# RazonIn4K/image-restoration-platform

Hardware: AMD Instinct MI355X
Metric: restored images/sec @1024x1024 bs=8 (higher is better)
Workload: dtype bf16; 1 GPU; 1024x1024 RGB u8, batch 8 per GPU: fused classifier scan + RestoreNet-v0 (43 convs, 779.9 GFLOP/image), seeded random-init weights; global_batch=8, parallelism=per-image data parallel x1, no collective, streams=1

## Files before the change

### image_restoration_platform_amd/build.py

```python
import concurrent.futures
import os
import subprocess
import sys

HERE = os.path.dirname(os.path.abspath(__file__))
CSRC = os.path.join(HERE, "csrc")
OBJ = os.path.join(HERE, "build")
LIB = os.path.join(HERE, "lib", "libire.so")

SOURCES = [
    ("classifier.hip", ["-ffp-contract=off"] + (["-DCLS_ABL=" + os.environ["CLS_ABL"]] if os.environ.get("CLS_ABL") else [])),
    ("conv_mfma.hip", []),
    ("conv_rb.hip", (["-DIRE_RB_ABLATE"] if os.environ.get("IRE_RB_ABLATE") else []) +
     (["-DIRE_RB_NGP64=" + os.environ["IRE_RB_NGP64"]] if os.environ.get("IRE_RB_NGP64") else [])),
    ("conv_w4.hip", (["-DIRE_W4_STAMPS"] if os.environ.get("IRE_RB_ABLATE") else []) +
     (["-DIRE_W4_TICKS"] if os.environ.get("IRE_RB_ABLATE") == "2" else []) +
     (["-DW4_TEPI=" + os.environ["IRE_W4_TEPI"]] if os.environ.get("IRE_W4_TEPI") else []) +
     (["-DIRE_W4_TL"] if os.environ.get("IRE_W4_TL") else [])),
    ("conv_up.hip", (["-DIRE_UP_ABL=" + os.environ["IRE_UP_ABL"]] if os.environ.get("IRE_UP_ABL") else []) +
     (["-DIRE_UP_D=" + os.environ["IRE_UP_D"]] if os.environ.get("IRE_UP_D") else []) +
     (["-DIRE_UP_TEPI=" + os.environ["IRE_UP_TEPI"]] if os.environ.get("IRE_UP_TEPI") else [])),
    ("conv_upq.hip", os.environ.get("UQ_DEFS", "").split()),
    ("conv_dnq.hip", os.environ.get("DQ_DEFS", "").split()),
    ("conv_down.hip", (["-DDN_LD_NT=" + os.environ["DN_LD_NT"]] if os.environ.get("DN_LD_NT") else [])),
    ("conv_stem.hip", []),
    ("conv_f8.hip", []),
    ("conv_pc.hip", (["-DC3_ABL=" + os.environ["C3_ABL"]] if os.environ.get("C3_ABL") else []) +
     (["-DC3_PRIO=" + os.environ["C3_PRIO"]] if os.environ.get("C3_PRIO") else []) +
     (["-DC3_RES_PRE=" + os.environ["C3_RES_PRE"]] if os.environ.get("C3_RES_PRE") else []) +
     (["-DC3_TEPI=" + os.environ["C3_TEPI"]] if os.environ.get("C3_TEPI") else []) +
     (["-DC3_TEPI64=" + os.environ["C3_TEPI64"]] if os.environ.get("C3_TEPI64") else []) +
     (["-DIRE_LD_ONCE32=" + os.environ["IRE_LD_ONCE32"]] if os.environ.get("IRE_LD_ONCE32") else []) +
     (["-DC3_PROD8=" + os.environ["C3_PROD8"]] if os.environ.get("C3_PROD8") else []) +
     (["-DIRE_PC_TICKS"] if os.environ.get("IRE_RB_ABLATE") == "2" else []) + (["-DIRE_W4_TL"] if os.environ.get("IRE_W4_TL") else [])),
    ("conv_pk.hip", (["-DPK_ABL=" + os.environ["PK_ABL"]] if os.environ.get("PK_ABL") else []) +
     (["-DPK_TICKS"] if os.environ.get("PK_TICKS") else []) + (["-DIRE_W4_TL"] if os.environ.get("IRE_W4_TL") else []) + os.environ.get("PK_DEFS", "").split()),
    ("gn.hip", []),
    ("fusion.hip", (["-DFUSE_FL=" + os.environ["FUSE_FL"]] if os.environ.get("FUSE_FL") else [])),
    ("preprocess.hip", []),
    ("encode.hip", []),
    ("deflate.hip", []),
    ("jpeg.hip", []),
    ("jpeg_dec.hip", []),
    ("engine.cpp", []),
    ("strips.cpp", []),
    ("api.cpp", []),
]
COMMON = ["--offload-arch=gfx950", "-O3", "-std=c++17", "-fPIC", "-Wall", "-Wno-unused-function",
          "-D__HIP_PLATFORM_AMD__"] + ([] if os.environ.get("IRE_SLP") == "1" else ["-fno-slp-vectorize"]) + \
         (["-DIRE_ST_LINE=" + os.environ["IRE_ST_LINE"]] if os.environ.get("IRE_ST_LINE") else []) + \
         (["-DIRE_ST_PART=" + os.environ["IRE_ST_PART"]] if os.environ.get("IRE_ST_PART") else []) + \
         (["-DIRE_LD_ONCE=" + os.environ["IRE_LD_ONCE"]] if os.environ.get("IRE_LD_ONCE") else []) + \
         (["-DIRE_LD_IN=" + os.environ["IRE_LD_IN"]] if os.environ.get("IRE_LD_IN") else []) + \
         os.environ.get("IRE_XFLAGS", "").split()

def _hipcc():
    for c in (os.environ.get("HIPCC"), "/opt/rocm/bin/hipcc", "hipcc"):
        if c and (os.path.isabs(c) and os.path.exists(c) or not os.path.isabs(c)):
            return c
    raise RuntimeError("hipcc not found")


def _deps_mtime():
    m = 0.0
    for root, _, files in os.walk(CSRC):
        for f in files:
# ... 94 lines not shown
```

### image_restoration_platform_amd/csrc/conv_mfma.hpp

```cpp
#pragma once
#include "common.hpp"
#include "conv_kind.hpp"

#ifndef IRE_ST_LINE
#define IRE_ST_LINE 16
#endif
#ifndef IRE_LD_ONCE
#define IRE_LD_ONCE 2
#endif
#ifndef IRE_LD_IN
#define IRE_LD_IN 0
#endif
#ifndef IRE_ST_PART
#define IRE_ST_PART 0
#endif

#include <cstdlib>

namespace ire {

inline int persistent_grid_cus() {
    static const int forced = [] { const char* v = std::getenv("IRE_GRID_CUS"); return v ? std::atoi(v) : 0; }();
    int dev = 0, cus = 256;
    (void)hipGetDevice(&dev);
// ... 8 lines not shown
    const void* in1;
    int cin0, cin1;
    int kc_split;
    int nkc;
    const unsigned short* w;
    const unsigned short* w1;
    const float* bias;
    const float2* ab;
    const float* gn_stats;
    int gn_parts, gn_hw;
    const float* gn_gamma;
    const float* gn_beta;
    const float* gn_film;
    int gn_film_stride, gn_film_off;
    float2* ab_w;
    const unsigned short* resid;
    unsigned short* out;
    const unsigned char* u8_in;
    unsigned char* u8_out;
    float* stats;
    int Hin, Win, Hout, Wout, cout;
    int tiles_x, tiles_y, nimg, nblocks;
    int group_size;
    int prio_young;
    int in_rows;
    int in_row_off;
    int iy_lo, iy_span;
    int fp8;
    const float* oscale;
    int w4_nt;
    const void* zeros;
    unsigned long long* stamps;
    int walk_rev;
};

void conv_launch(ConvKind kind, const ConvArgs& a, hipStream_t stream);

void conv_rb_launch(bool resid, bool fused_act, const ConvArgs& a, hipStream_t stream);
void conv_w4_launch(bool resid, const ConvArgs& a, hipStream_t stream);
void conv_f8_launch(bool resid, const ConvArgs& a, hipStream_t stream);
void conv_stem_launch(const ConvArgs& a, hipStream_t stream);
void conv_down_launch(const ConvArgs& a, hipStream_t stream);
void conv_head_launch(const ConvArgs& a, hipStream_t stream);
void conv_pc_launch(bool resid, bool head, const ConvArgs& a, hipStream_t stream);
void conv_pk_launch(bool resid, const ConvArgs& a, hipStream_t stream);
void conv_up_subpixel_launch(const ConvArgs& a, hipStream_t stream);
void conv_upq_launch(const ConvArgs& a, hipStream_t stream);
void conv_dnq_launch(const ConvArgs& a, hipStream_t stream);
void conv_up_launch(const ConvArgs& a, hipStream_t stream);

}
```

### image_restoration_platform_amd/csrc/conv_pc.hip

```cpp
#include "conv_mfma.hpp"
#include "conv_plan.hpp"
#include "gn_fold.hpp"
#include "persist.hpp"

#include <type_traits>

namespace ire {

namespace {

typedef __bf16 bf16x8_t __attribute__((ext_vector_type(8)));
typedef __bf16 bf16x2_t __attribute__((ext_vector_type(2)));
typedef float f32x2_t __attribute__((ext_vector_type(2)));
typedef float f32x16_t __attribute__((ext_vector_type(16)));
typedef unsigned u32x4_t __attribute__((ext_vector_type(4)));

#ifndef C3_RES_PRE
#define C3_RES_PRE -1
#endif
#ifndef C3_SCALAR
#define C3_SCALAR 1
#endif
#ifndef C3_PRIO
#define C3_PRIO 1
#endif
#ifndef C3_TEPI
#define C3_TEPI 1
#endif
#ifndef IRE_LD_ONCE32
#define IRE_LD_ONCE32 2
#endif
#ifndef C3_TEPI64
#define C3_TEPI64 1
#endif
#ifndef C3_PROD8
#define C3_PROD8 0
#endif
#ifndef C3_INTERIOR
#define C3_INTERIOR 0
#endif
#ifndef C3_ABL
#define C3_ABL 0
#endif
constexpr int C3_CONS = 512, C3_PROD = 256, C3_THREADS = C3_CONS + C3_PROD;
constexpr int pc_prod(int C, bool head) { return (C3_PROD8 && C == 32 && !head) ? 512 : 256; }
constexpr int C3_TH = 16, C3_TW = 32, C3_IH = C3_TH + 2, C3_IW = C3_TW + 2;
constexpr int C3_IN_CHUNKS = C3_IH * C3_IW * 4;
constexpr int C3_P_ITERS = (C3_IN_CHUNKS + C3_PROD - 1) / C3_PROD;
constexpr int C3_IN_BYTES = C3_P_ITERS * C3_PROD * 16;
template <int C> struct PcCfg {
    static constexpr int NT = C < 64 ? 32 : 64;
    static constexpr int NBLK = C / NT;
    static constexpr int NKC = C / 32;
    static constexpr int NTL = NT / 32;
    static constexpr int W_STAGE = 36 * NT * 16;
    static constexpr int W_STAGE_CHUNKS = 36 * NT;
    static constexpr int W_LDS = NKC * W_STAGE;
    static constexpr int W_OFF = 2 * C3_IN_BYTES;
    static constexpr int BIAS_OFF = W_OFF + W_LDS;
    static constexpr int NCC = NT / 8;
    static constexpr int RED_OFF = BIAS_OFF + C * 4;
    static constexpr int RED_HALF = 8 * NCC * 4;
    static constexpr int COEF_IMGS = pc_coef_imgs(C);
    static constexpr int COEF_OFF = RED_OFF + 2 * RED_HALF * 4;
    static constexpr int HEAD_OFF = COEF_OFF + COEF_IMGS * C * 2 * 4;
    static constexpr int PATCH_OFF = HEAD_OFF + (C == 32 ? 8 * 2 * 2 * 96 : 0);
    static constexpr int CNT_OFF = PATCH_OFF + (C == 32 ? 8 * 2048 : 0);
    static constexpr int LDS = CNT_OFF + (C == 64 ? 16 : 0);
    static_assert(LDS <= 160 * 1024, "LDS");
};

__device__ __forceinline__ unsigned c3_pack(float a, float b) {
// ... 57 lines not shown
    const int n_items = cursor.my_items;
    if (n_items == 0) return;
    const int n_stages = n_items * NKC;
    tl(0);
    {
        const unsigned char* ws = reinterpret_cast<const unsigned char*>(a.w);
        const unsigned wl = (unsigned)(size_t)(__attribute__((address_space(3))) unsigned char*)smem + K::W_OFF;
        constexpr int PIECES = NKC * K::W_STAGE_CHUNKS / 64;
        static_assert((NKC * K::W_STAGE_CHUNKS) % 64 == 0, "whole wave-instructions");
        const int wv = __builtin_amdgcn_readfirstlane(wave);
        for (int p = wv; p < PIECES; p += THREADS / 64) c3_glds16(ws + ((size_t)p * 64 + lane) * 16, wl + p * 1024);
    }
    if (a.gn_stats) gn_fold(a, smem, cursor.first_img, cursor.last_img, 512, reinterpret_cast<float2*>(smem + K::COEF_OFF));
    tl(1);

    {
        if (tid < C) reinterpret_cast<float*>(smem + K::BIAS_OFF)[tid] = a.bias[tid];
        if constexpr (C == 64) { if (tid == 0) *reinterpret_cast<unsigned*>(smem + K::CNT_OFF) = 0u; }
        const int nim = cursor.last_img - cursor.first_img + 1;
        const float2* ab = a.ab + (size_t)cursor.first_img * C;
        float2* cd = reinterpret_cast<float2*>(smem + K::COEF_OFF);
        if (!a.gn_stats) for (int i = tid; i < nim * C; i += THREADS) cd[i] = ab[i];
    }
    asm volatile("s_waitcnt vmcnt(0)" ::: "memory");
    __syncthreads();
    tl(2);

    if (__builtin_amdgcn_readfirstlane(wave) >= 8) {
#if C3_PRIO
        if (C3_PRIO != 1 || C != 32 || HEAD) asm volatile("s_setprio %0" :: "n"(C3_PRIO));
#endif
        const int tp = tid - C3_CONS;
        const int c8 = tp & 3;
        int rel[P_ITERS], lds_off[P_ITERS];
        unsigned pyx[P_ITERS];
#pragma unroll
        for (int i = 0; i < P_ITERS; ++i) {
            const int q = tp + i * PROD;
            const int p = q >> 2;
            const int py = p / C3_IW, px = p - py * C3_IW;
            pyx[i] = ((unsigned)py << 8) | (unsigned)px;
            rel[i] = (py * a.Win + px) * (2 * C) + c8 * 16;
            lds_off[i] = (p * 4 + (c8 ^ ((p >> 2) & 3))) * 16;
        }
        uint4 R[P_ITERS];
        unsigned okbits = 0;
        float cA[8], cB[8];
        PersistStage ls = cursor.cur;
        auto load_chunk = [&](int i) __attribute__((always_inline)) {
            const PersistItem& lit = ls.it;
            const int oy1 = lit.ty * C3_TH - 1, ox1 = lit.tx * C3_TW - 1;
            const char* base = reinterpret_cast<const char*>(a.in0) + (size_t)lit.img * a.in_rows * a.Win * (2 * C) + ls.kc * 64;
            const __amdgpu_buffer_rsrc_t irsrc = __builtin_amdgcn_make_buffer_rsrc(const_cast<char*>(base), 0, a.in_rows * a.Win * (2 * C) - ls.kc * 64, 0x00020000);
            const int base_off = ((oy1 + a.in_row_off) * a.Win + ox1) * (2 * C);
            const int y_lo = max(a.iy_lo - oy1, 0), y_hi = min(a.iy_lo + a.iy_span - oy1, C3_IH);
            const int x_lo = max(-ox1, 0), x_hi = min(a.Win - ox1, C3_IW);
            const int py = (int)(pyx[i] >> 8), px = (int)(pyx[i] & 0xffu);
            const bool ok = (unsigned)(py - y_lo) < (unsigned)(y_hi - y_lo) && (unsigned)(px - x_lo) < (unsigned)(x_hi - x_lo);
            const unsigned off = ok ? (unsigned)(base_off + rel[i]) : 0xffffffffu;
            if constexpr (C3_ABL & 8) { R[i] = make_uint4(off, 0x3f803f80u, i, 0x3f803f80u); }
            else {
                const u32x4_t lv = __builtin_amdgcn_raw_buffer_load_b128(irsrc, off, 0, IRE_LD_IN);
                R[i] = make_uint4(lv.x, lv.y, lv.z, lv.w);
            }
            okbits = (okbits & ~(1u << i)) | (ok ? (1u << i) : 0u);
        };
        auto load_coeffs = [&](const PersistStage& st) __attribute__((always_inline)) {
            const float4* ab = reinterpret_cast<const float4*>(smem + K::COEF_OFF) + ((st.it.img - cursor.first_img) * C + st.kc * 32 + c8 * 8) / 2;
#pragma unroll
            for (int e = 0; e < 4; ++e) { const float4 v = ab[e]; cA[2 * e] = v.x; cB[2 * e] = v.y; cA[2 * e + 1] = v.z; cB[2 * e + 1] = v.w; }
        };
        auto transform_stage_v = [&](unsigned char* tile, auto interior_tag) __attribute__((always_inline)) {
            constexpr bool INTERIOR = decltype(interior_tag)::value;
            auto pair = [&](auto pp_tag) __attribute__((always_inline)) {
                constexpr int pp_ = decltype(pp_tag)::value, i = 2 * pp_;
                constexpr int NCH = i + 1 < P_ITERS ? 2 : 1;
                constexpr int NW = 4 * NCH, NV = 8 * NCH;
                constexpr int i1 = NCH == 2 ? i + 1 : i;
                const unsigned wds[8] = {R[i].x, R[i].y, R[i].z, R[i].w, R[i1].x, R[i1].y, R[i1].z, R[i1].w};
                unsigned o[8];
                if constexpr (C3_ABL & 1) {
#pragma unroll
                    for (int w = 0; w < NW; ++w) o[w] = wds[w];
                } else {
#if C3_SCALAR
                    float y[16], e[16];
#pragma unroll
                    for (int w = 0; w < NW; ++w) {
                        const int d = w & 3;
                        y[2 * w] = __builtin_fmaf(c3_lo(wds[w]), cA[2 * d], cB[2 * d]);
                        y[2 * w + 1] = __builtin_fmaf(c3_hi(wds[w]), cA[2 * d + 1], cB[2 * d + 1]);
                    }
#pragma unroll
                    for (int k = 0; k < NV; ++k) e[k] = y[k] * (-1.4426950408889634f);
                    __builtin_amdgcn_sched_barrier(0);
#pragma unroll
                    for (int k = 0; k < NV; ++k) e[k] = __builtin_amdgcn_exp2f(e[k]);
                    __builtin_amdgcn_sched_barrier(0);
#pragma unroll
                    for (int k = 0; k < NV; ++k) e[k] = e[k] + 1.0f;
                    __builtin_amdgcn_sched_barrier(0);
#pragma unroll
                    for (int k = 0; k < NV; ++k) e[k] = __builtin_amdgcn_rcpf(e[k]);
                    __builtin_amdgcn_sched_barrier(0);
#pragma unroll
                    for (int w = 0; w < NW; ++w) o[w] = c3_pack(y[2 * w] * e[2 * w], y[2 * w + 1] * e[2 * w + 1]);
#else
                    static_assert(NCH == 2, "the packed-f32 form handles whole pairs");
                    f32x2_t y[8], e[8];
#pragma unroll
                    for (int w = 0; w < 8; ++w) {
                        const int d = w & 3;
                        const f32x2_t x = {c3_lo(wds[w]), c3_hi(wds[w])};
                        const f32x2_t A = {cA[2 * d], cA[2 * d + 1]}, B = {cB[2 * d], cB[2 * d + 1]};
                        y[w] = __builtin_elementwise_fma(x, A, B);
                        e[w] = y[w] * (-1.4426950408889634f);
                    }
                    __builtin_amdgcn_sched_barrier(0);
#pragma unroll
                    for (int w = 0; w < 8; ++w) e[w] = f32x2_t{__builtin_amdgcn_exp2f(e[w].x), __builtin_amdgcn_exp2f(e[w].y)};
                    __builtin_amdgcn_sched_barrier(0);
#pragma unroll
                    for (int w = 0; w < 8; ++w) e[w] = e[w] + 1.0f;
                    __builtin_amdgcn_sched_barrier(0);
#pragma unroll
                    for (int w = 0; w < 8; ++w) e[w] = f32x2_t{__builtin_amdgcn_rcpf(e[w].x), __builtin_amdgcn_rcpf(e[w].y)};
                    __builtin_amdgcn_sched_barrier(0);
#pragma unroll
                    for (int w = 0; w < 8; ++w) { const f32x2_t sv = y[w] * e[w]; o[w] = c3_pack(sv.x, sv.y); }
#endif
                }
#pragma unroll
                for (int k = 0; k < NCH; ++k) {
                    uint4 ov = make_uint4(o[4 * k], o[4 * k + 1], o[4 * k + 2], o[4 * k + 3]);
                    if constexpr (!INTERIOR) {
                        const unsigned m = (okbits >> (i + k)) & 1u ? 0xffffffffu : 0u;
                        ov = make_uint4(o[4 * k] & m, o[4 * k + 1] & m, o[4 * k + 2] & m, o[4 * k + 3] & m);
                    }
                    *reinterpret_cast<uint4*>(tile + lds_off[i + k]) = ov;
                }
                load_chunk(i);
                if constexpr (NCH == 2) load_chunk(i + 1);
                __builtin_amdgcn_sched_barrier(0);
            };
            pair(std::integral_constant<int, 0>{}); pair(std::integral_constant<int, 1>{}); pair(std::integral_constant<int, 2>{});
            if constexpr (P_ITERS > 6) { pair(std::integral_constant<int, 3>{}); pair(std::integral_constant<int, 4>{}); }
        };
        unsigned past_last = 0u;
        {
            const int q = tp + (P_ITERS - 1) * PROD;
            past_last = (q >> 2) >= C3_IH * C3_IW ? (1u << (P_ITERS - 1)) : 0u;
        }
        auto transform_stage = [&](unsigned char* tile) __attribute__((always_inline)) {
            if constexpr (C3_INTERIOR) {
                if (__builtin_amdgcn_ballot_w64((okbits | past_last) != (1u << P_ITERS) - 1u) == 0) { transform_stage_v(tile, std::true_type{}); return; }
            }
            transform_stage_v(tile, std::false_type{});
        };
#pragma unroll
        for (int i = 0; i < P_ITERS; ++i) load_chunk(i);
        load_coeffs(ls);
        ls = cursor.next();
        transform_stage(smem);
        c3_barrier();
        for (int t = 0; t < n_stages; ++t) {
            stamp_item = t / NKC;
            stamp(3 * (t % NKC) + 0);
            load_coeffs(ls);
            ls = cursor.next();
            transform_stage(smem + ((t + 1) & 1) * C3_IN_BYTES);
            stamp(3 * (t % NKC) + 1);
            c3_barrier();
            stamp(3 * (t % NKC) + 2);
        }
        return;
    }

    int a_off[2][9];
#pragma unroll
    for (int m = 0; m < 2; ++m)
#pragma unroll
        for (int tap = 0; tap < 9; ++tap) {
            const int ky = tap / 3, kx = tap - ky * 3;
            const int p = (wave * 2 + m + ky) * C3_IW + r + kx;
            a_off[m][tap] = (p * 4 + (h ^ ((p >> 2) & 3))) * 16;
        }
    const unsigned char* wb = smem + K::W_OFF + (h * NT + r) * 16;
    const float* bias_lds = reinterpret_cast<const float*>(smem + K::BIAS_OFF);
    f32x16_t bias_acc;
    if constexpr (C == 32) {
#pragma unroll
        for (int i = 0; i < 16; ++i) bias_acc[i] = bias_lds[16 * (i >> 3) + 8 * h + (i & 7)];
    }
    float* red_base = reinterpret_cast<float*>(smem + K::RED_OFF);
    int st_img = -1, st_tile = 0, st_nb = 0, st_par = 0, red_par = 0;
    auto flush_stats = [&]() {
        if (HEAD || st_img < 0) return;
        constexpr int G = C / 8, NGL = NT / G, CPG = G / 8;
        if (tid < NGL) {
            const float* red = red_base + st_par * K::RED_HALF;
            float s = 0.f, q = 0.f;
#pragma unroll
            for (int w = 0; w < 8; ++w) {
// ... 418 lines not shown
```

### image_restoration_platform_amd/csrc/engine.cpp

```cpp
#include "engine.hpp"
#include "encode.hpp"
#include "deflate.hpp"
#include "jpeg.hpp"
#include "jpeg_dec.hpp"

#include <chrono>
#include <cmath>
#include <cstdlib>
#include <cstring>
#include <fstream>

#include "gn.hpp"
#include "strips.hpp"
#include "weight_pack.hpp"
#include "grey_tables.inc"

namespace ire {

namespace {

inline double now_s() {
    return std::chrono::duration<double>(std::chrono::steady_clock::now().time_since_epoch()).count();
}

}

Engine::Engine(const ire_config& cfg) {
    int ndev = 0;
    hipError_t e = hipGetDeviceCount(&ndev);
    if (e != hipSuccess || ndev <= 0)
        fail(IRE_ERR_UNAVAILABLE, "service unavailable: no HIP device visible (the engine has no CPU fallback)");
    device_ = cfg.device_index;
    if (device_ < 0 || device_ >= ndev) fail(IRE_ERR_INVALID_INPUT, "invalid device_index");
    IRE_HIP(hipSetDevice(device_));
    hipDeviceProp_t prop;
    IRE_HIP(hipGetDeviceProperties(&prop, device_));
    if (std::strncmp(prop.gcnArchName, "gfx950", 6) != 0)
        fail(IRE_ERR_UNAVAILABLE, std::string("service unavailable: device is ") + prop.gcnArchName +
                                      ", this engine is built for gfx950 (MI355X) only");
    if (cfg.precision != IRE_PRECISION_BF16 && cfg.precision != IRE_PRECISION_FP8) fail(IRE_ERR_INVALID_INPUT, "invalid precision");
    precision_ = cfg.precision;
    max_batch_ = cfg.max_batch > 0 ? cfg.max_batch : 8;
    if (max_batch_ > 64) fail(IRE_ERR_INVALID_INPUT, "invalid max_batch (1..64)");
    num_lanes_ = cfg.num_streams > 0 ? cfg.num_streams : 1;
    if (num_lanes_ > 16) num_lanes_ = 16;
    if (cfg.flags & ~(uint32_t)(IRE_FLAG_RESULT_PNG_BASE64 | IRE_FLAG_RESULT_PNG_DEFLATE | IRE_FLAG_RESULT_JPEG))
        fail(IRE_ERR_INVALID_INPUT, "invalid ire_config.flags (unknown bits set)");
    if ((cfg.flags & (cfg.flags - 1)) != 0) fail(IRE_ERR_INVALID_INPUT, "invalid ire_config.flags (two result formats set)");
    flags_ = cfg.flags;
    sw_ = ConvSwitches::from_env();
    cus_ = persistent_grid_cus();
    if (const char* v = std::getenv("IRE_SNAKE")) snake_ = std::atoi(v) != 0;
    if (const char* v = std::getenv("IRE_JPEG_DEC_TIMES")) dec_times_ = std::atoi(v) != 0;
    if (const char* v = std::getenv("IRE_RB_STAMPS")) {
        stamps_cout_ = std::atoi(v);
        stamps_resid_ = std::strchr(v, 'r') != nullptr;
    }
    if (const char* v = std::getenv("IRE_W4_TL")) stamps_tl_ = v;

    IRE_HIP(hipStreamCreateWithFlags(&main_stream_, hipStreamNonBlocking));
    for (auto& ev : ev_) IRE_HIP(hipEventCreate(&ev));
    IRE_HIP(hipEventCreateWithFlags(&fork_ev_, hipEventDisableTiming));
    IRE_HIP(hipEventCreateWithFlags(&busy_ev_, hipEventDisableTiming));
    lanes_.resize(num_lanes_);
    for (auto& L : lanes_) {
        IRE_HIP(hipStreamCreateWithFlags(&L.stream, hipStreamNonBlocking));
        IRE_HIP(hipEventCreateWithFlags(&L.done, hipEventDisableTiming));
    }

    unsigned int* d_lin = tables_mem_.alloc<unsigned int>(sizeof(kLin16));
    unsigned int* d_thr = tables_mem_.alloc<unsigned int>(sizeof(kGreyThr));
    unsigned char* d_inv = tables_mem_.alloc<unsigned char>(5008);
    IRE_HIP(hipMemset(d_inv, 0, 5008));
    IRE_HIP(hipMemcpy(d_lin, kLin16, sizeof(kLin16), hipMemcpyHostToDevice));
    IRE_HIP(hipMemcpy(d_thr, kGreyThr, sizeof(kGreyThr), hipMemcpyHostToDevice));
    IRE_HIP(hipMemcpy(d_inv, kGreyInv, sizeof(kGreyInv), hipMemcpyHostToDevice));
    tables_ = ClassifierTables{d_lin, d_thr, d_inv};
    if (stamps_cout_) {
        stamps_dev_.grow(8 * 2 * 64 * 10 * 8);
        IRE_HIP(hipMemset(stamps_dev_.get<void>(), 0, 8 * 2 * 64 * 10 * 8));
    }

    if (cfg.weights_path && cfg.weights_path[0]) load_weights_file(cfg.weights_path);
}

// ... 593 lines not shown
    site.lin = op.lin; site.lout = op.lout; site.use_ab = op.use_ab; site.has_in1 = op.in1 != BUF_NONE; site.stats_out = op.stats_out;
    site.nimg = g.nimg; site.h = g.h; site.w = g.w; site.H = g.H; site.halo = g.halo; site.has_up = g.has_up; site.has_down = g.has_down;
    site.y0 = g.y0; site.cus = cus_;
    const ConvPlan p = plan_conv(sw_, d, site, precision_ == IRE_PRECISION_FP8);

    auto in_ptr = [&](int id) -> const unsigned short* { return id == BUF_NONE ? nullptr : g.buf[id >> 3][id & 7]; };
    auto out_ptr = [&](int id) -> unsigned short* {
        if (id == BUF_NONE) return nullptr;
        const int l = id >> 3;
        return g.buf[l][id & 7] + (size_t)g.halo * (g.w >> l) * kWidths[l];
    };
    const int Hout = g.h >> op.lout, Wout = g.w >> op.lout;
    ConvArgs a{};
    a.in0 = (d.kind == CONV_STEM) ? (const void*)g.img_in : (const void*)in_ptr(op.in0);
    a.in1 = in_ptr(op.in1);
    if (p.in1_first_row) a.in1 = in_ptr(op.in1) + (size_t)g.halo * Wout * d.cout;
    a.cin0 = d.cin0; a.cin1 = p.cin1; a.kc_split = d.kc_split; a.nkc = p.nkc; a.nblocks = p.nblocks; a.w4_nt = p.w4_nt; a.fp8 = p.fp8;
    const unsigned short* const slabs[] = {nullptr, cw.d_w, cw.d_wp, cw.d_w4, cw.d_w4h, cw.d_wstem, cw.d_wd, cw.d_wu, cw.d_wuf, cw.d_wdq, cw.d_wuq, cw.d_wsq,
                                           cw.d_wsk, reinterpret_cast<const unsigned short*>(cw.d_w8x), reinterpret_cast<const unsigned short*>(cw.d_w8)};
    const float* const biases[] = {cw.d_bias, cw.d_bias_uf, cw.d_bias8};
    a.w = slabs[p.w]; a.w1 = slabs[p.w1]; a.bias = biases[p.bias];
    if (p.fp8) a.oscale = cw.d_oscale;
    if (p.zeros) a.zeros = d_zero_.get<void>();
    a.ab = op.use_ab ? R.ab : nullptr; a.resid = out_ptr(op.resid); a.out = out_ptr(op.out);
    a.u8_in = d.kind == CONV_HEAD ? g.img_in + (size_t)g.halo * g.w * 3 : nullptr;
    a.u8_out = d.kind == CONV_HEAD ? g.img_out : nullptr;
    a.Hin = g.h >> op.lin; a.Win = g.w >> op.lin; a.Hout = Hout; a.Wout = Wout;
    a.in_rows = p.in_rows; a.in_row_off = p.in_row_off; a.iy_lo = p.iy_lo; a.iy_span = p.iy_span;
    a.cout = p.cout; a.group_size = p.group_size; a.tiles_x = p.tiles_x; a.tiles_y = p.tiles_y; a.nimg = g.nimg;
    if (op.stats_out) a.stats = (R.stats_alt ? R.stats_alt : R.stats) + p.stats_offset();
    a.prio_young = sw_.prio_young;
    a.walk_rev = R.snake && R.next_rev && p.kernel != K_V1;
    R.next_rev = !a.walk_rev;
    const bool rb = d.kind == CONV_RB1 || d.kind == CONV_RB2;
    if (stamps_dev_ && rb && d.cout == stamps_cout_ && (d.kind == CONV_RB2) == stamps_resid_ && (!stamps_taken_ || !stamps_tl_.empty() || std::getenv("IRE_STAMPS_RAW"))) {
        a.stamps = stamps_dev_.get<unsigned long long>();
        stamps_taken_ = true;
    }
    if (R.gn_pending) {
        if (p.folds_gn) {
            const GNW& gn = *R.gn_pending;
            a.gn_stats = R.gn_stats; a.gn_parts = R.gn_parts; a.gn_hw = (g.H >> gn.level) * (g.w >> gn.level);
            a.gn_gamma = gn.d_gamma; a.gn_beta = gn.d_beta; a.gn_film = R.film; a.gn_film_stride = kFilmDim; a.gn_film_off = kFilmOff[gn.level];
            a.ab_w = R.ab;
            R.gn_pending = nullptr;
        } else flush_gn(R, g);
    }
    prof_begin(p.fam, R.stream, p.flops, p.bytes);
    switch (p.kernel) {
        case K_V1: conv_launch(d.kind, a, R.stream); break;
        case K_F8: conv_f8_launch(p.resid, a, R.stream); break;
        case K_PK: conv_pk_launch(p.resid, a, R.stream); break;
        case K_W4: conv_w4_launch(p.resid, a, R.stream); break;
        case K_PC: conv_pc_launch(p.resid, false, a, R.stream); break;
        case K_RB: conv_rb_launch(p.resid, p.fused_act, a, R.stream); break;
        case K_PC_HEAD: conv_pc_launch(false, true, a, R.stream); break;
        case K_RB_HEAD: conv_head_launch(a, R.stream); break;
        case K_DNQ: conv_dnq_launch(a, R.stream); break;
        case K_DOWN: conv_down_launch(a, R.stream); break;
        case K_STEM: conv_stem_launch(a, R.stream); break;
        case K_UPQ: conv_upq_launch(a, R.stream); break;
        case K_UP_FUSED:
        case K_UP_SUB: conv_up_subpixel_launch(a, R.stream); break;
        case K_UP_RB: conv_up_launch(a, R.stream); break;
    }
    prof_tag(p.key, p.kname, op.lout, d.cin, d.cout, p.flops_exec);
// ... 4 lines not shown
    }
    if (capture_ && !op.name.empty() && a.out && g.halo == 0) capture(op.name.c_str(), a.out, (size_t)g.nimg * Hout * Wout * d.cout, R.stream);
    if (capture_ && !op.name.empty() && a.out && g.halo == 1)
        capture_rows(op.name.c_str(), a.out, (size_t)Hout * Wout * d.cout, (size_t)(g.H >> op.lout) * Wout * d.cout,
                     (size_t)(g.y0 >> op.lout) * Wout * d.cout, R.stream);
    if (capture_ && a.ab != nullptr && g.halo == 0)
        capture_f32(((op.name.empty() ? std::string("head") : op.name) + ".ab").c_str(), reinterpret_cast<const float*>(R.ab), (size_t)g.nimg * d.cin * 2, R.stream);
}

void Engine::flush_gn(Run& R, const Geo& g) {
    const GNW& gn = *R.gn_pending;
    prof_begin(FAM_GN, R.stream, 0, 0);
    gn_finalize_launch(R.gn_stats, g.nimg, R.gn_parts, gn.C, (g.H >> gn.level) * (g.w >> gn.level), gn.d_gamma, gn.d_beta, R.film, kFilmDim,
                       kFilmOff[gn.level], R.ab, R.stream);
    prof_end(R.stream);
    R.gn_pending = nullptr;
}

void Engine::exec_op(Run& R, const Op& op, const Geo& g) {
    switch (op.kind) {
        case Op::GN: {
            R.gn_pending = op.gn; R.gn_stats = R.stats; R.gn_parts = R.stat_parts;
            if (!sw_.gn_fold || g.halo) flush_gn(R, g);
            break;
        }
        case Op::CONV: exec_conv(R, op, g); break;
    }
}

void Engine::run_network(Lane& L, int nimg, int h, int w, const uint8_t* d_in, uint8_t* d_out, const float* d_film) {
    Run R;
    R.stream = L.stream; R.stats = L.v.stats; R.stats_alt = L.v.stats2; R.ab = L.v.ab; R.film = d_film;
    R.snake = snake_;
    const Geo g = geo_of_lane(L, nimg, h, w, d_in, d_out);
    prof_chain_ = false;
    prof_chainable_ = capture_ == false;
    prof_skip_ = prof_on_ == 2 && prof_every_ > 1 && (prof_pass_ % prof_every_) != 0;
    ++prof_pass_;
    for (const Op& op : program_) exec_op(R, op, g);
    prof_chainable_ = false;
    prof_chain_ = false;
    prof_skip_ = false;
}

void Engine::classify_device(const uint8_t* d_rgb, int n, int h, int w, const uint8_t* d_is_jpeg, double* d_scores,
                             int32_t* d_label, hipStream_t stream) {
    check_shape(n, h, w, false);
    if (!d_rgb) fail(IRE_ERR_INVALID_INPUT, "invalid input: null image pointer");
    ensure_io(n, 1, 1);
    prof_begin(FAM_CLASSIFIER, stream, 0, (double)n * h * w * 3);
    classifier_launch(tables_, d_rgb, n, h, w, d_is_jpeg, io_.sums, d_scores ? d_scores : io_.scores, d_label ? d_label : io_.label,
                      io_.cond, stream);
    prof_end(stream);
    last_n_ = n;
}

void Engine::restore_device(const uint8_t* d_rgb, int n, int h, int w, const double* d_scores, const uint8_t* d_is_jpeg,
                            uint8_t* d_out, hipStream_t stream) {
    check_shape(n, h, w, true);
    if (!net_.loaded) fail(IRE_ERR_UNAVAILABLE, "service unavailable: RestoreNet weights are not loaded");
    if (!d_rgb || !d_out) fail(IRE_ERR_INVALID_INPUT, "invalid input: null image pointer");
    ensure_io(n, 1, 1);
    ensure_workspace(n, h, w);
    if (d_scores) {
        scores_to_cond_launch(d_scores, n, io_.cond, stream);
    } else {
// ... 201 lines not shown
```

### image_restoration_platform_amd/csrc/engine.hpp

```cpp
#pragma once
#include <deque>
#include <map>
#include <memory>
#include <mutex>
#include <string>
#include <vector>

#include "classifier.hpp"
#include "common.hpp"
#include "conv_mfma.hpp"
#include "conv_plan.hpp"
#include "device_buf.hpp"

namespace ire {

struct PackedConv;
struct ConvW {
    ConvDesc desc;
    unsigned short* d_w = nullptr;
    unsigned short* d_wp = nullptr;
    unsigned short* d_w4 = nullptr;
    unsigned short* d_w4h = nullptr;
    unsigned short* d_wstem = nullptr;
    unsigned short* d_wd = nullptr;
// ... 36 lines not shown
    float2* ab = nullptr;
};
struct Lane {
    hipStream_t stream = nullptr;
    hipEvent_t done = nullptr;
    LaneBufs v;
};

constexpr int BUF_NONE = -1;
inline int buf_id(int level, int slot) { return level * 8 + slot; }
struct Op {
    enum Kind { GN, CONV } kind = CONV;
    const GNW* gn = nullptr;
    const ConvW* cw = nullptr;
    int in0 = BUF_NONE, in1 = BUF_NONE, resid = BUF_NONE, out = BUF_NONE;
    int lin = 0, lout = 0;
    bool use_ab = false;
    bool halo_out = false;
    bool stats_out = false;
    std::string name;
};
struct Run {
    hipStream_t stream = nullptr;
    float* stats = nullptr;
    float2* ab = nullptr;
    const float* film = nullptr;
    int stat_parts = 0;
    float* stats_alt = nullptr;
    const GNW* gn_pending = nullptr;
    const float* gn_stats = nullptr;
    int gn_parts = 0;
    bool snake = false;
    bool next_rev = false;
};
struct Geo {
    int nimg = 1, h = 0, w = 0;
    int halo = 0;
    bool has_up = false, has_down = false;
    int y0 = 0, H = 0;
    unsigned short* buf[4][6] = {};
    const uint8_t* img_in = nullptr;
    uint8_t* img_out = nullptr;
};

struct ProfRec {
    int fam;
    bool own_e0 = true;
    hipEvent_t e0, e1;
    double flops, bytes;
    double flops_exec = 0;
    int group = -1;
};
struct ProfGroup {
    std::string key, kernel;
    int level = 0, cin = 0, cout = 0;
    double ms = 0, flops = 0, flops_exec = 0, bytes = 0;
    int64_t n = 0;
};

class Engine {
    friend class StripSession;
public:
    explicit Engine(const ire_config& cfg);
    ~Engine();

    void load_weights(const void* blob, size_t bytes);
// ... 74 lines not shown
    void ensure_enc_scratch(size_t need, size_t full);
    uint8_t* ensure_enc_io(size_t need);
    void encode_deflate_window(const uint8_t* d_rgb, int n, int h, int w, size_t row_pitch, size_t image_pitch, uint8_t* d_chars, size_t stride, uint8_t* d_lens,
                               size_t lens_pitch, hipStream_t s);
    void encode_jpeg_window(const uint8_t* d_rgb, int n, int h, int w, size_t row_pitch, size_t image_pitch, uint8_t* d_chars, size_t stride, uint8_t* d_lens,
                            size_t lens_pitch, hipStream_t s);
    void encode_result(const uint8_t* d_rgb, int n, int h, int w, size_t row_pitch, size_t image_pitch, uint8_t* d_txt, size_t txt_stride, hipStream_t s);
    void ensure_io(int n, int h, int w);
    void ensure_workspace(int n, int h, int w);
    void free_workspace();
    void build_program();
    void run_network(Lane& L, int nimg, int h, int w, const uint8_t* d_in, uint8_t* d_out, const float* d_film);
    void exec_op(Run& R, const Op& op, const Geo& g);
    void flush_gn(Run& R, const Geo& g);
    void exec_conv(Run& R, const Op& op, const Geo& g);
    static Geo geo_of_lane(const Lane& L, int nimg, int h, int w, const uint8_t* d_in, uint8_t* d_out);
    void prof_begin(int fam, hipStream_t s, double flops, double bytes);
    void prof_tag(const char* key, const char* kernel, int level, int cin, int cout, double flops_exec);
    void prof_end(hipStream_t s);
    void capture(const char* name, const unsigned short* d, size_t count, hipStream_t s);
    void capture_rows(const char* name, const unsigned short* d, size_t count, size_t total, size_t offset, hipStream_t s);
    void capture_f32(const char* name, const float* d, size_t count, hipStream_t s);
    template <class T> T* upload(const std::vector<T>& v);
    ConvW upload_conv(const PackedConv& p);

    int device_ = 0;
    int max_batch_ = 8;
    int num_lanes_ = 1;
    uint32_t flags_ = 0;
    int precision_ = IRE_PRECISION_BF16;
    ConvSwitches sw_;
    int cus_ = 256;
    bool snake_ = true;
    std::mutex mu_;
    hipStream_t main_stream_ = nullptr;
    hipEvent_t ev_[4] = {};
    hipEvent_t fork_ev_ = nullptr;
    hipEvent_t busy_ev_ = nullptr;
    bool busy_recorded_ = false;
    int64_t batches_run_ = 0, images_restored_ = 0;
    int last_batch_ = 0;
    std::deque<std::pair<double, int>> recent_;
    double t0_ = 0.0;

    ClassifierTables tables_{};
    BufSet<DeviceMem> tables_mem_;

    IoBufs<DeviceMem> io_;
    int last_n_ = 0;
    FuseBufs<DeviceMem> fuse_;
    Buf<DeviceMem> d_zero_;
    Buf<DeviceMem> d_pp_tab_, d_pp_mid_, d_pp_in_, d_pp_out_;
    Buf<DeviceMem> d_enc_scratch_;
    Buf<DeviceMem> d_pad_in_, d_pad_out_;
    Buf<DeviceMem> d_enc_io_;
    Buf<PinnedMem> dec_pin_[2];
    Buf<DeviceMem> d_dec_in_, d_dec_coef_, d_dec_planes_, d_dec_out_;
    hipEvent_t dec_up_ev_[2] = {};
    bool dec_up_recorded_[2] = {};
    int dec_turn_ = 0;
    bool dec_times_ = false, dec_marks_pending_ = false;
    hipEvent_t dec_marks_[6] = {};
    double dec_ms_[5] = {};
    int64_t dec_calls_ = 0;
    void dec_times_collect();

// ... 34 lines not shown
```

### image_restoration_platform_amd/csrc/persist.hpp

```cpp
#pragma once

#if defined(__HIPCC__) || defined(__CUDACC__)
#define IRE_HD __host__ __device__ __forceinline__
#else
#define IRE_HD inline
#endif

namespace ire {

struct PersistItem { int img, ty, tx, nb, tile; };
struct PersistStage { PersistItem it; int kc; };

struct PersistCursor {
    int S;
    int my_items;
    int nkc, nblocks, tiles_x, tiles_y;
    int d_img, d_ty, d_tx, d_nb;
    int s;
    PersistStage cur;
    int first_img, last_img;

    IRE_HD PersistCursor(int tiles_x_, int tiles_y_, int nimg, int nblocks_, int nkc_, int G, int block, bool reverse) {
        tiles_x = tiles_x_; tiles_y = tiles_y_; nblocks = nblocks_; nkc = nkc_;
        const int tiles_per_img = tiles_x * tiles_y;
        const int items = tiles_per_img * nimg * nblocks;
        const int X = G < 8 ? G : 8;
        const int xcd = block % X, jx = block / X;
        const int nwx = (G - xcd + X - 1) / X;
        const int lo = (int)((long long)items * xcd / X), hi = (int)((long long)items * (xcd + 1) / X);
        my_items = (lo + jx < hi) ? (hi - lo - jx + nwx - 1) / nwx : 0;
        S = my_items * nkc;
        auto split = [&](int L, int& img, int& ty, int& tx, int& nb) {
            nb = L % nblocks;
            const int t = L / nblocks;
            img = t / tiles_per_img;
            const int tile = t - img * tiles_per_img;
            ty = tile / tiles_x;
            tx = tile - ty * tiles_x;
        };
        split(nwx, d_img, d_ty, d_tx, d_nb);
        const int L_lo = lo + jx, span = my_items > 0 ? (my_items - 1) * nwx : 0;
        split(reverse ? L_lo + span : L_lo, cur.it.img, cur.it.ty, cur.it.tx, cur.it.nb);
        cur.it.tile = cur.it.ty * tiles_x + cur.it.tx;
        cur.kc = 0;
// ... 33 lines not shown
```

Baseline: 1105 images/sec.

## Reuse overlapping halo rows from previous tile in persistent 3x3 conv

When the persistent cursor's next tile is the vertical neighbour of the previous one (same image, column and output block), the two shared halo rows are copied LDS-to-LDS from the prior stage buffer instead of being reloaded from global memory and retransformed. The producer slot mapping is permuted so the shared rows land in the last round of loads, which is then split between fresh transform and copy across producer waves. This cuts global traffic and transform work for the overlapping rows. It adds extra LDS traffic and branching, depends on the walk order, and the old interior fast path is removed (with an optional padding-fix variant). Enabled by default, with a kill switch via environment variable.

Result: no change. 1109 images/sec, median of 6 (+0.4%).

```diff
diff --git a/image_restoration_platform_amd/build.py b/image_restoration_platform_amd/build.py
--- a/image_restoration_platform_amd/build.py
+++ b/image_restoration_platform_amd/build.py
@@ -32,6 +32,8 @@
      (["-DC3_TEPI64=" + os.environ["C3_TEPI64"]] if os.environ.get("C3_TEPI64") else []) +
      (["-DIRE_LD_ONCE32=" + os.environ["IRE_LD_ONCE32"]] if os.environ.get("IRE_LD_ONCE32") else []) +
      (["-DC3_PROD8=" + os.environ["C3_PROD8"]] if os.environ.get("C3_PROD8") else []) +
+     (["-DC3_HALO_REUSE=" + os.environ["C3_HALO_REUSE"]] if os.environ.get("C3_HALO_REUSE") else []) +
+     (["-DC3_PADFIX=" + os.environ["C3_PADFIX"]] if os.environ.get("C3_PADFIX") else []) +
      (["-DIRE_PC_TICKS"] if os.environ.get("IRE_RB_ABLATE") == "2" else []) + (["-DIRE_W4_TL"] if os.environ.get("IRE_W4_TL") else [])),
     ("conv_pk.hip", (["-DPK_ABL=" + os.environ["PK_ABL"]] if os.environ.get("PK_ABL") else []) +
      (["-DPK_TICKS"] if os.environ.get("PK_TICKS") else []) + (["-DIRE_W4_TL"] if os.environ.get("IRE_W4_TL") else []) + os.environ.get("PK_DEFS", "").split()),
diff --git a/image_restoration_platform_amd/csrc/conv_mfma.hpp b/image_restoration_platform_amd/csrc/conv_mfma.hpp
--- a/image_restoration_platform_amd/csrc/conv_mfma.hpp
+++ b/image_restoration_platform_amd/csrc/conv_mfma.hpp
@@ -64,6 +64,7 @@
     const void* zeros;
     unsigned long long* stamps;
     int walk_rev;
+    int halo_reuse;
 };
 
 void conv_launch(ConvKind kind, const ConvArgs& a, hipStream_t stream);
diff --git a/image_restoration_platform_amd/csrc/conv_pc.hip b/image_restoration_platform_amd/csrc/conv_pc.hip
--- a/image_restoration_platform_amd/csrc/conv_pc.hip
+++ b/image_restoration_platform_amd/csrc/conv_pc.hip
@@ -36,8 +36,11 @@
 #ifndef C3_PROD8
 #define C3_PROD8 0
 #endif
-#ifndef C3_INTERIOR
-#define C3_INTERIOR 0
+#ifndef C3_HALO_REUSE
+#define C3_HALO_REUSE 1
+#endif
+#ifndef C3_PADFIX
+#define C3_PADFIX 0
 #endif
 #ifndef C3_ABL
 #define C3_ABL 0
@@ -161,21 +164,38 @@
 #endif
         const int tp = tid - C3_CONS;
         const int c8 = tp & 3;
+        constexpr bool REUSE = C3_HALO_REUSE && NKC == 1 && PROD == 256;
+        constexpr int FRESH = C3_TH * C3_IW * 4, SHARED_PIX = 2 * C3_IW;
+        static_assert((C3_TH * C3_IW) % 16 == 0, "the shared rows' LDS swizzle phase is the same at both ends of a tile");
+        const bool reuse_on = REUSE && a.halo_reuse != 0;
+        const bool rows_fwd = reuse_on && a.walk_rev == 0;
         int rel[P_ITERS], lds_off[P_ITERS];
         unsigned pyx[P_ITERS];
+        unsigned real_bits = 0, shared_bits = 0;
 #pragma unroll
         for (int i = 0; i < P_ITERS; ++i) {
             const int q = tp + i * PROD;
-            const int p = q >> 2;
+            int p = q >> 2;
+            if (REUSE && rows_fwd) p = q < FRESH ? p + SHARED_PIX : q < C3_IN_CHUNKS ? p - FRESH / 4 : p;
             const int py = p / C3_IW, px = p - py * C3_IW;
             pyx[i] = ((unsigned)py << 8) | (unsigned)px;
             rel[i] = (py * a.Win + px) * (2 * C) + c8 * 16;
             lds_off[i] = (p * 4 + (c8 ^ ((p >> 2) & 3))) * 16;
-        }
+            if (q < C3_IN_CHUNKS) real_bits |= 1u << i;
+            if (REUSE && q >= FRESH && q < C3_IN_CHUNKS) shared_bits |= 1u << i;
+        }
+        int cp_off = 0;
+        if constexpr (REUSE) {
+            const int cq = tp >= PROD / 2 ? tp - PROD / 2 : tp + PROD;
+            const int pd = (cq >> 2) + (rows_fwd ? 0 : FRESH / 4);
+            cp_off = (pd * 4 + (c8 ^ ((pd >> 2) & 3))) * 16;
+        }
+        const int cp_src = rows_fwd ? FRESH * 16 : -FRESH * 16;
         uint4 R[P_ITERS];
         unsigned okbits = 0;
         float cA[8], cB[8];
         PersistStage ls = cursor.cur;
+        bool skip_ld = false;
         auto load_chunk = [&](int i) __attribute__((always_inline)) {
             const PersistItem& lit = ls.it;
             const int oy1 = lit.ty * C3_TH - 1, ox1 = lit.tx * C3_TW - 1;
@@ -185,7 +205,8 @@
             const int y_lo = max(a.iy_lo - oy1, 0), y_hi = min(a.iy_lo + a.iy_span - oy1, C3_IH);
             const int x_lo = max(-ox1, 0), x_hi = min(a.Win - ox1, C3_IW);
             const int py = (int)(pyx[i] >> 8), px = (int)(pyx[i] & 0xffu);
-            const bool ok = (unsigned)(py - y_lo) < (unsigned)(y_hi - y_lo) && (unsigned)(px - x_lo) < (unsigned)(x_hi - x_lo);
+            bool ok = (unsigned)(py - y_lo) < (unsigned)(y_hi - y_lo) && (unsigned)(px - x_lo) < (unsigned)(x_hi - x_lo);
+            if (REUSE && i >= FRESH / PROD) ok = ok && !(skip_ld && ((shared_bits >> i) & 1u));
             const unsigned off = ok ? (unsigned)(base_off + rel[i]) : 0xffffffffu;
             if constexpr (C3_ABL & 8) { R[i] = make_uint4(off, 0x3f803f80u, i, 0x3f803f80u); }
             else {
@@ -199,11 +220,8 @@
 #pragma unroll
             for (int e = 0; e < 4; ++e) { const float4 v = ab[e]; cA[2 * e] = v.x; cB[2 * e] = v.y; cA[2 * e + 1] = v.z; cB[2 * e + 1] = v.w; }
         };
-        auto transform_stage_v = [&](unsigned char* tile, auto interior_tag) __attribute__((always_inline)) {
-            constexpr bool INTERIOR = decltype(interior_tag)::value;
-            auto pair = [&](auto pp_tag) __attribute__((always_inline)) {
-                constexpr int pp_ = decltype(pp_tag)::value, i = 2 * pp_;
-                constexpr int NCH = i + 1 < P_ITERS ? 2 : 1;
+        auto xform = [&](unsigned char* tile, auto i_tag, auto nch_tag) __attribute__((always_inline)) {
+                constexpr int i = decltype(i_tag)::value, NCH = decltype(nch_tag)::value;
                 constexpr int NW = 4 * NCH, NV = 8 * NCH;
                 constexpr int i1 = NCH == 2 ? i + 1 : i;
                 const unsigned wds[8] = {R[i].x, R[i].y, R[i].z, R[i].w, R[i1].x, R[i1].y, R[i1].z, R[i1].w};
@@ -262,42 +280,66 @@
 #pragma unroll
                 for (int k = 0; k < NCH; ++k) {
                     uint4 ov = make_uint4(o[4 * k], o[4 * k + 1], o[4 * k + 2], o[4 * k + 3]);
-                    if constexpr (!INTERIOR) {
+                    if constexpr (!C3_PADFIX) {
                         const unsigned m = (okbits >> (i + k)) & 1u ? 0xffffffffu : 0u;
                         ov = make_uint4(o[4 * k] & m, o[4 * k + 1] & m, o[4 * k + 2] & m, o[4 * k + 3] & m);
                     }
                     *reinterpret_cast<uint4*>(tile + lds_off[i + k]) = ov;
                 }
+        };
+        auto transform_stage = [&](unsigned char* tile, const unsigned char* other, bool reuse) __attribute__((always_inline)) {
+            const unsigned pad = ~okbits & (REUSE && reuse ? real_bits & ~shared_bits : real_bits);
+            auto pair = [&](auto pp_tag) __attribute__((always_inline)) {
+                constexpr int pp_ = decltype(pp_tag)::value, i = 2 * pp_;
+                constexpr int NCH = i + 1 < P_ITERS ? 2 : 1;
+                if constexpr (REUSE && i + NCH > FRESH / PROD) {
+                    static_assert(i == FRESH / PROD && NCH == 2 && 2 * FRESH / PROD == 2 * i + 1, "round 8 is half fresh, round 9 has no fresh slot");
+                    const int pw = __builtin_amdgcn_readfirstlane(wave) - C3_CONS / 64;
+                    if (!reuse) xform(tile, std::integral_constant<int, i>{}, std::integral_constant<int, 2>{});
+                    else {
+                        if (pw < 2) xform(tile, std::integral_constant<int, i>{}, std::integral_constant<int, 1>{});
+                        if (pw >= 2) {
+                            const uint4 v0 = *reinterpret_cast<const uint4*>(other + cp_off + cp_src);
+                            const uint4 v1 = *reinterpret_cast<const uint4*>(other + cp_off + cp_src + 32 * 64);
+                            *reinterpret_cast<uint4*>(tile + cp_off) = v0;
+                            *reinterpret_cast<uint4*>(tile + cp_off + 32 * 64) = v1;
+                        } else if (pw == 0 && tp < SHARED_PIX * 4 - PROD) {
+                            *reinterpret_cast<uint4*>(tile + cp_off) = *reinterpret_cast<const uint4*>(other + cp_off + cp_src);
+                        }
+                    }
+                } else xform(tile, std::integral_constant<int, i>{}, std::integral_constant<int, NCH>{});
                 load_chunk(i);
                 if constexpr (NCH == 2) load_chunk(i + 1);
                 __builtin_amdgcn_sched_barrier(0);
             };
             pair(std::integral_constant<int, 0>{}); pair(std::integral_constant<int, 1>{}); pair(std::integral_constant<int, 2>{});
             if constexpr (P_ITERS > 6) { pair(std::integral_constant<int, 3>{}); pair(std::integral_constant<int, 4>{}); }
-        };
-        unsigned past_last = 0u;
-        {
-            const int q = tp + (P_ITERS - 1) * PROD;
-            past_last = (q >> 2) >= C3_IH * C3_IW ? (1u << (P_ITERS - 1)) : 0u;
-        }
-        auto transform_stage = [&](unsigned char* tile) __attribute__((always_inline)) {
-            if constexpr (C3_INTERIOR) {
-                if (__builtin_amdgcn_ballot_w64((okbits | past_last) != (1u << P_ITERS) - 1u) == 0) { transform_stage_v(tile, std::true_type{}); return; }
-            }
-            transform_stage_v(tile, std::false_type{});
+            if constexpr (C3_PADFIX) {
+                if (__builtin_amdgcn_ballot_w64(pad != 0u) != 0) {
+#pragma unroll
+                    for (int i = 0; i < P_ITERS; ++i)
+                        if ((pad >> i) & 1u) *reinterpret_cast<uint4*>(tile + lds_off[i]) = make_uint4(0u, 0u, 0u, 0u);
+                }
+            }
         };
 #pragma unroll
         for (int i = 0; i < P_ITERS; ++i) load_chunk(i);
         load_coeffs(ls);
-        ls = cursor.next();
-        transform_stage(smem);
+        auto step = [&]() __attribute__((always_inline)) {
+            const PersistItem prev = ls.it;
+            ls = cursor.next();
+            if constexpr (REUSE) skip_ld = reuse_on && persist_vertical_neighbour(prev, ls.it, a.walk_rev != 0);
+        };
+        step();
+        transform_stage(smem, smem + C3_IN_BYTES, false);
         c3_barrier();
         for (int t = 0; t < n_stages; ++t) {
             stamp_item = t / NKC;
             stamp(3 * (t % NKC) + 0);
             load_coeffs(ls);
-            ls = cursor.next();
-            transform_stage(smem + ((t + 1) & 1) * C3_IN_BYTES);
+            const bool reuse = skip_ld;
+            step();
+            transform_stage(smem + ((t + 1) & 1) * C3_IN_BYTES, smem + (t & 1) * C3_IN_BYTES, reuse);
             stamp(3 * (t % NKC) + 1);
             c3_barrier();
             stamp(3 * (t % NKC) + 2);
diff --git a/image_restoration_platform_amd/csrc/engine.cpp b/image_restoration_platform_amd/csrc/engine.cpp
--- a/image_restoration_platform_amd/csrc/engine.cpp
+++ b/image_restoration_platform_amd/csrc/engine.cpp
@@ -51,6 +51,7 @@
     sw_ = ConvSwitches::from_env();
     cus_ = persistent_grid_cus();
     if (const char* v = std::getenv("IRE_SNAKE")) snake_ = std::atoi(v) != 0;
+    if (const char* v = std::getenv("IRE_HALO_REUSE")) halo_reuse_ = std::atoi(v) != 0;
     if (const char* v = std::getenv("IRE_JPEG_DEC_TIMES")) dec_times_ = std::atoi(v) != 0;
     if (const char* v = std::getenv("IRE_RB_STAMPS")) {
         stamps_cout_ = std::atoi(v);
@@ -710,6 +711,7 @@
     a.prio_young = sw_.prio_young;
     a.walk_rev = R.snake && R.next_rev && p.kernel != K_V1;
     R.next_rev = !a.walk_rev;
+    a.halo_reuse = R.halo_reuse && p.kernel != K_V1;
     const bool rb = d.kind == CONV_RB1 || d.kind == CONV_RB2;
     if (stamps_dev_ && rb && d.cout == stamps_cout_ && (d.kind == CONV_RB2) == stamps_resid_ && (!stamps_taken_ || !stamps_tl_.empty() || std::getenv("IRE_STAMPS_RAW"))) {
         a.stamps = stamps_dev_.get<unsigned long long>();
@@ -780,6 +782,7 @@
     Run R;
     R.stream = L.stream; R.stats = L.v.stats; R.stats_alt = L.v.stats2; R.ab = L.v.ab; R.film = d_film;
     R.snake = snake_;
+    R.halo_reuse = halo_reuse_;
     const Geo g = geo_of_lane(L, nimg, h, w, d_in, d_out);
     prof_chain_ = false;
     prof_chainable_ = capture_ == false;
diff --git a/image_restoration_platform_amd/csrc/engine.hpp b/image_restoration_platform_amd/csrc/engine.hpp
--- a/image_restoration_platform_amd/csrc/engine.hpp
+++ b/image_restoration_platform_amd/csrc/engine.hpp
@@ -92,6 +92,7 @@
     int gn_parts = 0;
     bool snake = false;
     bool next_rev = false;
+    bool halo_reuse = false;
 };
 struct Geo {
     int nimg = 1, h = 0, w = 0;
@@ -232,6 +233,7 @@
     ConvSwitches sw_;
     int cus_ = 256;
     bool snake_ = true;
+    bool halo_reuse_ = true;
     std::mutex mu_;
     hipStream_t main_stream_ = nullptr;
     hipEvent_t ev_[4] = {};
diff --git a/image_restoration_platform_amd/csrc/persist.hpp b/image_restoration_platform_amd/csrc/persist.hpp
--- a/image_restoration_platform_amd/csrc/persist.hpp
+++ b/image_restoration_platform_amd/csrc/persist.hpp
@@ -10,6 +10,10 @@
 
 struct PersistItem { int img, ty, tx, nb, tile; };
 struct PersistStage { PersistItem it; int kc; };
+
+IRE_HD bool persist_vertical_neighbour(const PersistItem& prev, const PersistItem& next, bool reverse) {
+    return next.img == prev.img && next.tx == prev.tx && next.nb == prev.nb && next.ty == prev.ty + (reverse ? -1 : 1);
+}
 
 struct PersistCursor {
     int S;
```
